# wenlinlee/FISCO-BCOS

Measured on AMD Instinct MI355X. Metric: sigs_per_sec, higher is better.
Workload: dtype u32 (256-bit integer); 1 GPU; C2; txs_total=10000, txs_rank0=10000, parallelism=dp1 (tx-index shards)

## Files before the change

### fisco-bcos_amd/csrc/ecc_coop.hip

```cpp
#include "ecc_device.h"
#include "ec26_trio.h"

namespace bcosgpu {

struct SplitLds {
    uint32_t tab[8][16][64];
    uint32_t zc[8][64];
    uint32_t u1[8][64];
    uint32_t k1[4][64];
    uint32_t k2[4][64];
    uint32_t flags[64];
    uint32_t pt[3][25][64];
};

__device__ __forceinline__ void lds_store_jac(uint32_t (*dst)[64], const Jac& P, int lane) {
    lds_store_fe(dst, P.X, lane);
    lds_store_fe(dst + 8, P.Y, lane);
    lds_store_fe(dst + 16, P.Z, lane);
    dst[24][lane] = P.inf ? 1u : 0u;
}
__device__ __forceinline__ void lds_load_jac(Jac& P, const uint32_t (*src)[64], int lane) {
    lds_load_fe(P.X, src, lane);
    lds_load_fe(P.Y, src + 8, lane);
    lds_load_fe(P.Z, src + 16, lane);
    P.inf = src[24][lane] != 0u;
}

__device__ __forceinline__ void add_digit_lds(Jac& acc, const SplitLds& L, int lane, int d, bool neg, bool phi) {
    const uint32_t m = static_cast<uint32_t>((d < 0 ? -d : d) - 1) & 7u;
    const uint32_t* base = &L.tab[0][0][0] + m * (16 * 64) + lane;
    Aff S;
#pragma unroll
    for (int k = 0; k < 8; ++k) {
        S.x.v[k] = base[k * 64];
        S.y.v[k] = base[(8 + k) * 64];
    }
    if (phi) {
        fe b;
        fe_set(b, kGlvBeta);
        FieldK1::mul(S.x, S.x, b);
    }
    fe ny;
    FieldK1::neg(ny, S.y);
    fe_cmov(S.y, ny, (d < 0) != neg);
    Jac R;
    CurveK1::madd(R, acc, S);
    CurveK1::cmov(acc, R, d != 0);
}

__device__ __forceinline__ void glv_half_lds(Jac& acc, fe& k, bool neg, bool phi, const SplitLds& L, int lane) {
    CurveK1::set_inf(acc);
    add_digit_lds(acc, L, lane, static_cast<int>(k.v[3] >> 31), neg, phi);
#pragma unroll 1
    for (int i = 31; i >= 0; --i) {
        CurveK1::dbl(acc, acc);
        CurveK1::dbl(acc, acc);
        CurveK1::dbl(acc, acc);
        CurveK1::dbl(acc, acc);
        add_digit_lds(acc, L, lane, booth_digit128(k), neg, phi);
    }
}

__global__ __launch_bounds__(256, 1) void tx_verify_split_kernel(const uint8_t* __restrict__ pre,
                                                                 const uint64_t* __restrict__ pre_off,
                                                                 const uint8_t* __restrict__ sig,
                                                                 const uint64_t* __restrict__ sig_off, uint64_t n,
                                                                 const uint32_t* __restrict__ tab,
                                                                 uint8_t* __restrict__ txhash,
                                                                 uint8_t* __restrict__ sender,
                                                                 uint8_t* __restrict__ status) {
    __shared__ SplitLds L;
    const int wave = threadIdx.x >> 6, lane = threadIdx.x & 63;
    const uint64_t i = static_cast<uint64_t>(blockIdx.x) * 64 + lane;
    const bool active = i < n;
    uint64_t sa = 0, sb = 0;
    if (active) {
        sa = sig_off[i];
        sb = sig_off[i + 1];
    }
    const uint32_t slen = (sb - sa) > 0xffffffffull ? 0xffffffffu : static_cast<uint32_t>(sb - sa);
    if (wave == 1) {
        if (active) {
            const uint64_t a = pre_off[i], b = pre_off[i + 1];
            const uint32_t len = static_cast<uint32_t>(b - a);
            ByteReader rd(pre + a, len);
            uint32_t d[8];
            keccak256_msg(rd, len, d);
            store_digest(KECCAK256, txhash + 32 * i, d);
            fe e, r, s;
            uint32_t v;
            fe_from_be_words(e, d);
            reduce_once(e, ParamN1::M);
            const bool ok = parse_sig65(sig + sa, slen, r, s, v);
            if (!ok) {
                fe_zero(r);
                r.v[0] = 1;
                fe_zero(s);
            }
            fe rm, rinv, u1, u2, k1, k2;
            FieldN1::from_plain(rm, r);
            FieldInv<FieldN1>::inv(rinv, rm);
            FieldN1::mul(u1, e, rinv);
            FieldN1::neg(u1, u1);
            FieldN1::mul(u2, s, rinv);
            bool neg1, neg2;
            glv_split(k1, neg1, k2, neg2, u2);
            lds_store_fe(L.u1, u1, lane);
#pragma unroll
            for (int k = 0; k < 4; ++k) {
                L.k1[k][lane] = k1.v[k];
                L.k2[k][lane] = k2.v[k];
            }
            L.flags[lane] = (ok ? 1u : 0u) | (neg1 ? 4u : 0u) | (neg2 ? 8u : 0u);
        }
    } else if (wave == 2) {
        if (active) {
            fe r, s;
            uint32_t v;
            bool ok = parse_sig65(sig + sa, slen, r, s, v);
            fe x;
            fe_copy(x, r);
            if (v & 2u) {
                ok = ok && fe_lt_k(r, kK1PminusN);
                fe_add_k(x, r, ParamN1::M);
            }
            fe rhs, y, t, seven;
            FieldK1::sqr(t, x);
            FieldK1::mul(rhs, t, x);
            fe_zero(seven);
            seven.v[0] = 7;
            FieldK1::add(rhs, rhs, seven);
            FieldK1::sqrt_cand(y, rhs);
            FieldK1::sqr(t, y);
            ok = ok && FieldK1::eq(t, rhs);
            FieldK1::normalize(y);
            fe ny;
            FieldK1::neg(ny, y);
            FieldK1::normalize(ny);
            fe_cmov(y, ny, (y.v[0] & 1u) != (v & 1u));
            Aff R, A[8];
            fe_copy(R.x, x);
            fe_copy(R.y, y);
            fe Zc;
            {
                Jac T[8];
                multiples8<CurveK1>(T, R);
                coz_table_k1(A, Zc, T);
            }
            Unroll<0, 8>::run([&](auto J) {
                constexpr int j = decltype(J)::value;
                lds_store_fe(L.tab[j], A[j].x, lane);
                lds_store_fe(L.tab[j] + 8, A[j].y, lane);
            });
            lds_store_fe(L.zc, Zc, lane);
            L.pt[2][24][lane] = ok ? 2u : 0u;
        }
    }
    __syncthreads();
    uint32_t flags = 0;
    if (active) flags = L.flags[lane] | L.pt[2][24][lane];
    __syncthreads();
    if (wave <= 1) {
        if (active) {
            fe k;
            fe_zero(k);
#pragma unroll
            for (int q = 0; q < 4; ++q) k.v[q] = wave == 0 ? L.k1[q][lane] : L.k2[q][lane];
            const bool neg = wave == 0 ? (flags & 4u) != 0 : (flags & 8u) != 0;
            Jac P;
            glv_half_lds(P, k, neg, wave == 1, L, lane);
            lds_store_jac(L.pt[wave], P, lane);
        }
    } else if (wave == 2) {
        if (active) {
            fe u1;
            lds_load_fe(u1, L.u1, lane);
            Jac PG;
            comb_mul<CurveK1, 8>(PG, u1, tab);
            lds_store_jac(L.pt[2], PG, lane);
        }
    }
    __syncthreads();
    if (wave == 0 && active) {
        Jac P0, P1, PG, Q, R;
        lds_load_jac(P0, L.pt[0], lane);
        lds_load_jac(P1, L.pt[1], lane);
        lds_load_jac(PG, L.pt[2], lane);
        fe Zc;
        lds_load_fe(Zc, L.zc, lane);
        CurveK1::add(Q, P0, P1);
        FieldK1::mul(Q.Z, Q.Z, Zc);
        CurveK1::add(R, Q, PG);
        const bool ok = (flags & 3u) == 3u && !R.inf;
        Aff A;
        CurveK1::to_aff(A, R);
        FieldK1::normalize(A.x);
        FieldK1::normalize(A.y);
        uint32_t ad[5] = {0, 0, 0, 0, 0};
        if (ok) keccak_address(ad, A.x, A.y);
        uint32_t* o = reinterpret_cast<uint32_t*>(sender + 20 * i);
#pragma unroll
        for (int k = 0; k < 5; ++k) o[k] = ad[k];
        status[i] = ok ? 0 : 1;
    }
}

#ifdef BCOSGPU_COOP_TIMING
__device__ uint64_t g_coop_t[8][12];
__device__ uint64_t g_dbl_t[4][8];
#define DBL_T(k) \
    if (c.probe && (threadIdx.x & 63) == 0) g_dbl_t[threadIdx.x >> 6][k] = clock64()
#define COOP_T(k) \
    if (blockIdx.x == 0 && (threadIdx.x & 63) == 0) g_coop_t[threadIdx.x >> 6][k] = clock64()
#else
#define COOP_T(k) \
    do {          \
    } while (0)
#define DBL_T(k) \
    do {         \
    } while (0)
#endif
struct CoopLds {
    uint32_t tab[8][16][64];
    uint32_t zc[8][64];
    uint32_t k[2][4][64];
    uint32_t flags[64];
    uint4 ex[2][2][6][2][64];
    uint32_t tabphx[8][8][64];
    uint32_t pt[5][25][64];
    uint32_t xe[8][64];
    uint32_t xrinv[8][64];
    uint32_t ys[8][64];
    uint32_t rflag[64];
    uint32_t post[2];
};

struct CoopCtx {
    CoopLds* L;
    int chain, role, lane;
    bool probe;
    __device__ __forceinline__ uint4* slot(int x, int r, int f) const {
        return &L->ex[chain][r][x == 0 ? f : 2 + x][0][0] + lane;
    }
    __device__ __forceinline__ void put(int x, int f, const fe& a) const {
        uint4* p = slot(x, role, f);
        p[0] = make_uint4(a.v[0], a.v[1], a.v[2], a.v[3]);
        p[64] = make_uint4(a.v[4], a.v[5], a.v[6], a.v[7]);
    }
    __device__ __forceinline__ void puts(int s, const fe& a) const {
        uint4* p = &L->ex[chain][role][s][0][0] + lane;
        p[0] = make_uint4(a.v[0], a.v[1], a.v[2], a.v[3]);
        p[64] = make_uint4(a.v[4], a.v[5], a.v[6], a.v[7]);
    }
    __device__ __forceinline__ void gets(int s, fe& a) const {
        const uint4* p = &L->ex[chain][role ^ 1][s][0][0] + lane;
        const uint4 q0 = p[0], q1 = p[64];
        a.v[0] = q0.x; a.v[1] = q0.y; a.v[2] = q0.z; a.v[3] = q0.w;
        a.v[4] = q1.x; a.v[5] = q1.y; a.v[6] = q1.z; a.v[7] = q1.w;
    }
    __device__ __forceinline__ void get(int x, int f, fe& a) const {
        const uint4* p = slot(x, role ^ 1, f);
        const uint4 q0 = p[0], q1 = p[64];
        a.v[0] = q0.x; a.v[1] = q0.y; a.v[2] = q0.z; a.v[3] = q0.w;
        a.v[4] = q1.x; a.v[5] = q1.y; a.v[6] = q1.z; a.v[7] = q1.w;
    }
};

template <int S0>
__device__ __forceinline__ void coop_dbl(Jac& P, const CoopCtx& c) {
    fe E, F, D, C8, Z3, X3, Y3, t;
    DBL_T(0);
    if (c.role == 0) {
        fe A;
        FieldK1::sqr(A, P.X);
        FieldK1::mul3(E, A);
        FieldK1::sqr(F, E);
        c.puts(S0, E);
        c.puts(S0 + 1, F);
        FieldK1::mul(Z3, P.Y, P.Z);
        FieldK1::template shl<1>(Z3, Z3);
        c.puts(S0 + 2, Z3);
    } else {
        fe B, C;
        FieldK1::sqr(B, P.Y);
        FieldK1::mul(D, P.X, B);
        FieldK1::template shl<2>(D, D);
        c.puts(S0, D);
        FieldK1::sqr(C, B);
        FieldK1::template shl<3>(C8, C);
        c.puts(S0 + 1, C8);
    }
    DBL_T(1);
    __syncthreads();
    DBL_T(2);
    if (c.role == 0) {
        c.gets(S0, D);
        c.gets(S0 + 1, C8);
    } else {
        c.gets(S0, E);
        c.gets(S0 + 1, F);
        c.gets(S0 + 2, Z3);
    }
    FieldK1::template shl<1>(t, D);
    FieldK1::sub(X3, F, t);
// ... 829 lines not shown
    if (wave == 1) {
        fe u2, k1, k2;
        FieldN1::mul(u2, VERIFY ? r : s, rinv);
        bool neg1, neg2;
        glv_split(k1, neg1, k2, neg2, u2);
#pragma unroll
        for (int q = 0; q < 4; ++q) {
            L.k[0][q][lane] = k1.v[q];
            L.k[1][q][lane] = k2.v[q];
        }
        L.flags[lane] = (ok ? 1u : 0u) | (neg1 ? 4u : 0u) | (neg2 ? 8u : 0u);
    }
}

struct CombShare {
    int wide[4][2], narrow[4][2];
};
__device__ __forceinline__ void comb_share(int& lo, int& hi, const int (&t)[4][2], int wave) {
    lo = t[0][0];
    hi = t[0][1];
#pragma unroll
    for (int w = 1; w < 4; ++w) {
        if (wave == w) {
            lo = t[w][0];
            hi = t[w][1];
        }
    }
}
__device__ __forceinline__ void comb_share_range(Jac26& G, const fe& u1, const uint32_t* __restrict__ tab, int tab_bits,
                                                 const CombShare& share, int wave) {
    int lo, hi;
    if (tab_bits == kWideBits) {
        comb_share(lo, hi, share.wide, wave);
        comb_range26w<kWideBits>(G, u1, tab, lo, hi);
    } else {
        comb_share(lo, hi, share.narrow, wave);
        comb_range26w<8>(G, u1, tab, lo, hi);
    }
}
constexpr int kPairShare[4][2] = {{0, 12}, {24, 32}, {0, 0}, {12, 24}};
constexpr int kTrioSplitWin[3] = {5, 10, 16};
static_assert(0 < kTrioSplitWin[0] && kTrioSplitWin[0] < kTrioSplitWin[1] && kTrioSplitWin[1] < kTrioSplitWin[2] &&
                  kTrioSplitWin[2] <= 16,
              "comb windows of helpers 0, 1, 3, 2");
constexpr CombShare trio_recover_share() {
    const int a = kTrioSplitWin[0], b = kTrioSplitWin[1], c = kTrioSplitWin[2];
    return {{{0, a}, {a, b}, {c, 16}, {b, c}}, {{0, 2 * a}, {2 * a, 2 * b}, {2 * c, 32}, {2 * b, 2 * c}}};
}
constexpr CombShare kTrioRecoverShare = trio_recover_share();
constexpr CombShare kTrioVerifyShare = {{{0, 6}, {15, 16}, {10, 15}, {6, 10}}, {{0, 11}, {30, 32}, {19, 30}, {11, 19}}};

template <class LDS>
__device__ __forceinline__ void coop26_store_partial(LDS& L, const Jac26& G, int wave, int lane) {
    if (wave == 0) {
        coop26_store_jac(L.pt[2], G, lane);
        lds_flag_post(&L.post[2]);
    } else if (wave == 3) {
        Jac26 G0, S;
        lds_flag_wait(&L.post[2]);
        coop26_load_jac(G0, L.pt[2], lane);
        CurveK1x::add(S, G0, G);
        coop26_store_jac(L.pt[3], S, lane);
    } else {
        coop26_store_jac(L.pt[wave == 1 ? 4 : 0], G, lane);
    }
}

template <class IO>
__device__ __forceinline__ void coop26_body(const IO& io, uint64_t n, const uint32_t* __restrict__ tab) {
    __shared__ Coop26Lds L;
    const int wave = threadIdx.x >> 6, lane = threadIdx.x & 63;
    const uint64_t i = static_cast<uint64_t>(blockIdx.x) * 64 + lane;
    const bool active = i < n;
    COOP_T(0);
    if (threadIdx.x == 0) {
        L.post[0] = 0u;
        L.post[1] = 0u;
        L.post[2] = 0u;
    }
    __syncthreads();
    fe r, s;
    uint32_t v = 0;
    bool ok = false;
    if (active) ok = io.rsv(i, r, s, v);
    else { fe_zero(r); fe_zero(s); }
    if (wave == 1 || wave == 2) {
        fe26 X, rhs;
        bool okr = recover_w(X, rhs, r, v, ok);
        if (wave == 2) {
            fe26 y, ny, t;
            fe26_sqrt_cand(y, rhs);
            fe26_sqr(t, y);
            fe26_sub<3>(t, t, rhs);
            okr = okr && fe26_is_zero(t);
            fe26_normalize(y);
            fe26_neg<2>(ny, y);
            fe26_normalize(ny);
            fe26_cmov(y, ny, (y.v[0] & 1u) != (v & 1u));
            lds_store_fe26(L.ys, y, lane);
            L.rflag[lane] = okr ? 2u : 0u;
            COOP_T(6);
        } else {
            Aff26 R;
            fe26_mul(R.x, rhs, X);
            fe26_sqr(R.y, rhs);
            coop26_table_to_lds<false>(L, R, lane);
            COOP_T(6);
        }
    }
    coop26_post_e_inv<false, false>(L, io, i, active, ok, r, s, wave, lane);
    if (wave != 2) {
        fe u1;
        coop26_u1_glv<false>(u1, L, ok, r, s, wave, lane);
        Jac26 G;
        int lo, hi;
        comb_share(lo, hi, kPairShare, wave);
        comb_range26w<8>(G, u1, tab, lo, hi);
        coop26_store_partial(L, G, wave, lane);
    }
    COOP_T(1);
    __syncthreads();
    const uint32_t flags = L.flags[lane] | L.rflag[lane];
    {
        Coop26Ctx c{&L, wave >> 1, wave & 1, lane, false};
        fe k;
        fe_zero(k);
#pragma unroll
        for (int q = 0; q < 4; ++q) k.v[q] = L.k[c.chain][q][lane];
        const bool neg = c.chain == 0 ? (flags & 4u) != 0 : (flags & 8u) != 0;
        const bool phi = c.chain == 1;
        Jac26 acc;
        CurveK1x::set_inf(acc);
        coop26_add_digit(acc, c, static_cast<int>(k.v[3] >> 31), neg, phi);
#pragma unroll 1
        for (int w = 31; w >= 0; --w) {
            coop26_dbl<0>(acc, c);
#ifdef BCOSGPU_COOP_TIMING
            c.probe = blockIdx.x == 0 && w == 20;
#endif
            coop26_dbl<3>(acc, c);
#ifdef BCOSGPU_COOP_TIMING
            c.probe = false;
            if (blockIdx.x == 0 && w == 20 && (threadIdx.x & 63) == 0) g_dbl_t[threadIdx.x >> 6][5] = clock64();
#endif
            coop26_dbl<0>(acc, c);
            coop26_dbl<3>(acc, c);
#ifdef BCOSGPU_COOP_TIMING
            if (blockIdx.x == 0 && w == 20 && (threadIdx.x & 63) == 0) g_dbl_t[threadIdx.x >> 6][6] = clock64();
#endif
            coop26_add_digit(acc, c, booth_digit128(k), neg, phi);
#ifdef BCOSGPU_COOP_TIMING
            if (blockIdx.x == 0 && w == 20 && (threadIdx.x & 63) == 0) g_dbl_t[threadIdx.x >> 6][7] = clock64();
#endif
        }
        COOP_T(2);
        if (c.role == 0) coop26_store_jac(L.pt[c.chain], acc, lane);
    }
    __syncthreads();
    if (wave == 1) {
        Jac26 G01, G2, U;
        coop26_load_jac(G01, L.pt[3], lane);
        coop26_load_jac(G2, L.pt[4], lane);
        CurveK1x::add(U, G01, G2);
        coop26_store_jac(L.pt[2], U, lane);
    } else if (wave == 0) {
        Jac26 P0, P1, Q;
        coop26_load_jac(P0, L.pt[0], lane);
        coop26_load_jac(P1, L.pt[1], lane);
        fe26 Zc, y;
        lds_load_fe26(Zc, L.zc, lane);
        lds_load_fe26(y, L.ys, lane);
        CurveK1x::add(Q, P0, P1);
        fe26_mul(Zc, Zc, y);
        fe26_mul(Q.Z, Q.Z, Zc);
        coop26_store_jac(L.pt[0], Q, lane);
    }
    __syncthreads();
    if (wave == 0 && active) {
        Jac26 Q, G, R;
        coop26_load_jac(Q, L.pt[0], lane);
        coop26_load_jac(G, L.pt[2], lane);
        CurveK1x::add(R, Q, G);
        const bool ok2 = (flags & 3u) == 3u && !R.inf;
        COOP_T(4);
        fe z, zi, ax, ay;
        fe26_to_fe(z, R.Z);
        FieldInv<FieldK1>::inv(zi, z);
        COOP_T(5);
        fe26 zi26, zi2, zi3, X, Y;
        fe26_from_fe(zi26, zi);
        fe26_sqr(zi2, zi26);
        fe26_mul(X, R.X, zi2);
        fe26_mul(zi3, zi2, zi26);
        fe26_mul(Y, R.Y, zi3);
        fe26_to_fe(ax, X);
        fe26_to_fe(ay, Y);
        uint32_t ad[5] = {0, 0, 0, 0, 0};
        if (ok2 && io.want_addr()) keccak_address(ad, ax, ay);
        io.finish(i, ok2, ad, &ax, &ay);
    }
    COOP_T(3);
}

constexpr int kTrioTxs = 40;
struct TrioSeat {
    int chain, tl;
    bool real;
    __device__ __forceinline__ TrioSeat(int wave, int lane, const TrioLane& T) {
        const int trio_idx = (lane & 15) / 3;
        chain = wave & 1;
        tl = (wave >> 1) * 20 + (lane >> 4) * 5 + (trio_idx < 5 ? trio_idx : 4);
        real = T.r2 && trio_idx < 5;
    }
};

template <class IO>
__device__ __forceinline__ void trio_recover_tail(const IO& io, uint32_t* mbuf, int wave, int lane, const TrioSeat& seat,
                                                  uint64_t ti, bool tactive, bool ok2, const fe& ax, const fe& ay) {
    if (seat.chain == 0 && io.want_addr()) {
        const KeccakPair kp;
        const int j = lane >> 1, t = (wave >> 1) * 20 + (j < 20 ? j : 0);
        uint32_t d[4];
        kp.hash(reinterpret_cast<const uint8_t*>(mbuf + 16 * t), 64u, d);
        if (j < 20) {
#pragma unroll
            for (int q = 0; q < 4; ++q) mbuf[640 + 8 * t + 2 * q + (lane & 1)] = d[q];
        }
    }
    __syncthreads();
    if (seat.chain == 0 && seat.real && tactive) {
        uint32_t ad[5] = {0, 0, 0, 0, 0};
        if (ok2 && io.want_addr()) {
#pragma unroll
            for (int q = 0; q < 5; ++q) ad[q] = mbuf[640 + 8 * seat.tl + 3 + q];
        }
        io.finish(ti, ok2, ad, &ax, &ay);
    }
}

__device__ __forceinline__ void lds_flag_wait_idle(uint32_t* f) {
    while (__hip_atomic_load(f, __ATOMIC_ACQUIRE, __HIP_MEMORY_SCOPE_WORKGROUP) == 0u) __builtin_amdgcn_s_sleep(8);
}

template <class IO>
__device__ __forceinline__ void trio_recover_helper(Trio26RecoverLds& L, const IO& io, uint64_t i, bool active, bool ok,
                                                    const fe& r, uint32_t v, const uint32_t* __restrict__ tab, int tab_bits,
                                                    int h, int lane) {
    constexpr bool kRootAdds = kTrioSplitWin[2] < 16;
    constexpr int kLast = kRootAdds ? 3 : 2;
    if (h == 2) {
        fe26 X, w, y, ny, t;
        const bool okr = recover_w(X, w, r, v, ok);
        fe26_sqrt_cand(y, w);
        fe26_sqr(t, y);
        fe26_sub<3>(t, t, w);
        const bool on = fe26_is_zero(t);
        fe26_normalize(y);
        fe26_neg<2>(ny, y);
        fe26_normalize(ny);
        fe26_cmov(y, ny, (y.v[0] & 1u) != (v & 1u));
        if (lane < kTrioTxs) {
#pragma unroll
            for (int q = 0; q < 10; ++q) L.sq[q][lane] = y.v[q];
        }
        L.rflag[lane] = okr ? 2u : 0u;
        L.yok[lane] = on ? 1u : 0u;
        COOP_T(6);
    } else if (h == 3) {
        fe e;
        fe_zero(e);
        if (active) io.template digest<KECCAK256>(i, e);
        reduce_once(e, ParamN1::M);
        lds_store_fe(L.xe, e, lane);
        lds_flag_post(&L.post[1]);
        COOP_T(7);
    }
    int lo, hi;
    comb_share(lo, hi, kTrioRecoverShare.wide, h);
    if (lo != hi) {
        lds_flag_wait_idle(&L.post[0]);
        lds_flag_wait_idle(&L.post[1]);
        fe e, rinv, u1;
        lds_load_fe(e, L.xe, lane);
        lds_load_fe(rinv, L.xrinv, lane);
        FieldN1::mul(u1, e, rinv);
        FieldN1::neg(u1, u1);
        Jac26 G;
        comb_share_range(G, u1, tab, tab_bits, kTrioRecoverShare, h);
        const int j = h == 0 ? 0 : h == 1 ? 1 : h == 3 ? 2 : 3;
        if (j > 0) {
            Jac26 P, S;
            lds_flag_wait_idle(&L.hpost[j - 1]);
            coop26_load_jac(P, L.pt[j - 1], lane);
            CurveK1x::add(S, P, G);
            coop26_store_jac(L.pt[j == kLast ? 3 : j], S, lane);
        } else {
            coop26_store_jac(L.pt[0], G, lane);
        }
        if (j != kLast) lds_flag_post(&L.hpost[j]);
        COOP_T(10);
    }
}

template <class IO>
__device__ __forceinline__ void trio26_recover_body(const IO& io, uint64_t n, const uint32_t* __restrict__ tab,
                                                    int tab_bits) {
    __shared__ Trio26RecoverLds L;
    const int wave = __builtin_amdgcn_readfirstlane(static_cast<int>(threadIdx.x >> 6)), lane = threadIdx.x & 63;
    const bool helper = wave >= 4;
    const uint64_t i = static_cast<uint64_t>(blockIdx.x) * kTrioTxs + lane;
    const bool active = lane < kTrioTxs && i < n;
    COOP_T(0);
    if (threadIdx.x == 0) {
        L.post[0] = 0u;
        L.post[1] = 0u;
        L.post[2] = 0u;
#pragma unroll
        for (int q = 0; q < kTfSlots; ++q) L.spost[q] = 0u;
#pragma unroll
        for (int q = 0; q < 4; ++q) L.hpost[q] = 0u;
    }
    __syncthreads();
    const TrioLane T(lane);
    TrioSeat seat(wave, lane, T);
    if (helper) seat.chain = 2;
    const int chain = seat.chain, tl = seat.tl;
    uint32_t tflags = 0;
    TrioPt acc;
    {
        fe r, s;
        uint32_t v = 0;
        bool ok = false;
        fe_zero(r);
        fe_zero(s);
        if (active && (wave <= 3 || wave == 4 + 2)) ok = io.rsv(i, r, s, v);
        if (helper) {
            trio_recover_helper(L, io, i, active, ok, r, v, tab, tab_bits, wave - 4, lane);
            COOP_T(1);
        } else {
            if (wave == 0) {
                if (!ok) {
                    fe_zero(r);
                    r.v[0] = 1;
                    fe_zero(s);
                }
                fe rm, rinv, u2, k1, k2;
                FieldN1::from_plain(rm, r);
                FieldInv<FieldN1>::inv_pipe(rinv, rm);
                lds_store_fe(L.xrinv, rinv, lane);
                lds_flag_post(&L.post[0]);
                COOP_T(7);
                FieldN1::mul(u2, s, rinv);
                COOP_T(10);
                bool neg1, neg2;
                glv_split(k1, neg1, k2, neg2, u2);
                COOP_T(11);
#pragma unroll
                for (int q = 0; q < 4; ++q) {
                    L.k[0][q][lane] = k1.v[q];
                    L.k[1][q][lane] = k2.v[q];
                }
                L.flags[lane] = (ok ? 1u : 0u) | (neg1 ? 4u : 0u) | (neg2 ? 8u : 0u);
                lds_flag_post(&L.spost[0]);
                COOP_T(8);
            } else {
                fe26 X, rhs, beta;
                recover_w(X, rhs, r, v, ok);
                Aff26 R;
                fe26_mul(R.x, rhs, X);
                fe26_sqr(R.y, rhs);
                fe26_const(beta, kGlvBeta);
                TrioTableFlags tf{L.spost};
                if (wave == 1) trio_table_shared<kTableLong>(L, tf, R, rhs, beta, lane);
                else if (wave == 2) trio_table_shared<kTablePrefix>(L, tf, R, rhs, beta, lane);
                else trio_table_shared<kTableShort>(L, tf, R, rhs, beta, lane);
            }
            COOP_T(1);
            lds_flag_wait4(&L.spost[0], &L.spost[kTfDone[kTableLong]], &L.spost[kTfDone[kTablePrefix]],
                           &L.spost[kTfDone[kTableShort]]);
            COOP_T(9);
            tflags = L.flags[tl];
            trio_glv_chain(acc, L, chain, tl, tflags, T);
            COOP_T(2);
        }
    }
    uint32_t* const xbuf = &L.xg[(wave >> 1) & 1][0][0];
    uint32_t* const mbuf = &L.tabphx[0][0][0];
    const uint64_t ti = static_cast<uint64_t>(blockIdx.x) * kTrioTxs + tl;
    const bool tactive = ti < n;
    fe ax, ay;
    bool ok2 = false;
    const auto load_k = [&](fe26& K) {
#pragma unroll
        for (int q = 0; q < 10; ++q) K.v[q] = L.kw[q][tl];
        F26_SETM(K, 1);
    };
    const auto load_g = [&](TrioPt& G) {
        Jac26 J;
        coop26_load_jac(J, L.pt[3], tl);
        trio_from_jac(G, J, T);
    };
    TrioPt SE;
    fe26 zi2, zi3;
    fe26_zero(zi2);
    fe26_zero(zi3);
    if (chain == 1) {
        trio_store(xbuf, acc, lane);
        lds_flag_post(&L.spost[5 + (wave >> 1)]);
    } else if (chain == 0) {
        TrioPt P1;
        lds_flag_wait(&L.spost[5 + (wave >> 1)]);
        trio_load(P1, xbuf, lane);
        trio_add(acc, acc, P1, T);
        trio_store(xbuf, acc, lane);
        fe26 K;
        load_k(K);
        trio_scale_xz(SE, acc, K, T);
    }
    __syncthreads();
    const uint32_t rfl = L.rflag[tl];
    if (chain == 0) {
        TrioPt G;
        load_g(G);
        fe26 Z3;
        trio_add_z(Z3, G, SE, T);
        COOP_T(4);
        fe z, zi;
        fe26_to_fe(z, Z3);
        FieldInv<FieldK1>::inv_trio<2, 2>(zi, z, T, lane);
        COOP_T(5);
        fe26 zi26;
        fe26_from_fe(zi26, zi);
        fe26_sqr(zi2, zi26);
        fe26_mul(zi3, zi2, zi26);
    } else if (chain == 1) {
        TrioPt S, G;
        trio_load(S, xbuf, lane);
        load_g(G);
        fe26 y, zc, K, l;
        load_k(K);
        lds_load_fe26(zc, L.zc, tl);
        trio_scale_xz(SE, S, K, T);
#pragma unroll
        for (int q = 0; q < 10; ++q) y.v[q] = L.sq[q][tl];
        F26_SETM(y, 1);
        COOP_T(4);
        fe26_mul(l, zc, y);
        trio_scale_y(SE, l, T);
        trio_add(S, G, SE, T);
        trio_store(xbuf, S, lane);
        COOP_T(5);
    }
    __syncthreads();
    if (chain == 0) {
        TrioPt O;
        trio_load(O, xbuf, lane);
        ok2 = (tflags & 1u) != 0u && (rfl & 2u) != 0u && L.yok[tl] != 0u && !O.inf;
        fe26 X, Y;
        fe26_mul(X, O.Xs, zi2);
        fe26_mul(Y, O.S1, zi3);
        fe26_to_fe(ax, X);
        fe26_to_fe(ay, Y);
        if (seat.real) {
            uint32_t m[16];
            fe_to_be_words(m, ax);
            fe_to_be_words(m + 8, ay);
#pragma unroll
            for (int q = 0; q < 16; ++q) mbuf[16 * tl + q] = m[q];
        }
    }
    __syncthreads();
    trio_recover_tail(io, mbuf, wave, lane, seat, ti, tactive, ok2, ax, ay);
    COOP_T(3);
}

__device__ __forceinline__ void trio26_verify_body(const KeyIO& io, uint64_t n, const uint32_t* __restrict__ tab,
                                                   int tab_bits) {
    __shared__ Trio26Lds L;
    const int wave = threadIdx.x >> 6, lane = threadIdx.x & 63;
    const uint64_t i = static_cast<uint64_t>(blockIdx.x) * kTrioTxs + lane;
    const bool active = lane < kTrioTxs && i < n;
    COOP_T(0);
    if (threadIdx.x == 0) {
        L.post[0] = 0u;
        L.post[1] = 0u;
        L.post[2] = 0u;
    }
    __syncthreads();
    fe r, s;
    bool ok = false;
    {
        fe kx, ky;
        if (active) {
            io.key_rs(i, r, s, kx, ky);
            ok = fe_lt_k(kx, FieldK1::P) && fe_lt_k(ky, FieldK1::P) && !fe_is_zero_raw(r) && !fe_is_zero_raw(s) &&
                 fe_lt_k(r, ParamN1::M) && fe_lt_k(s, kN1HalfPlus);
        } else {
            fe_zero(r);
            fe_zero(s);
            fe_zero(kx);
            fe_zero(ky);
        }
        if (wave == 0) lds_store_fe(L.ys, r, lane);
        if (wave == 1) {
            Aff26 P;
            fe26_from_fe(P.x, kx);
            fe26_from_fe(P.y, ky);
            fe26 l, rr, t, seven;
            fe26_sqr(l, P.y);
            fe26_sqr(t, P.x);
            fe26_mul(rr, t, P.x);
            fe26_set_small(seven, 7u);
            fe26_add(rr, rr, seven);
            fe26_sub<3>(l, l, rr);
            const bool on = fe26_is_zero(l);
            if (!(ok && on)) {
                fe26_const(P.x, kK1Gx);
                fe26_const(P.y, kK1Gy);
            }
            L.rflag[lane] = on ? 2u : 0u;
            coop26_table_to_lds<true>(L, P, lane);
            COOP_T(6);
        }
    }
    coop26_post_e_inv<true, true>(L, io, i, active, ok, r, s, wave, lane);
    {
        fe u1;
        coop26_u1_glv<true>(u1, L, ok, r, s, wave, lane);
        Jac26 G;
        comb_share_range(G, u1, tab, tab_bits, kTrioVerifyShare, wave);
        coop26_store_partial(L, G, wave, lane);
    }
    COOP_T(1);
    __syncthreads();
    const TrioLane T(lane);
    const TrioSeat seat(wave, lane, T);
    const int chain = seat.chain, tl = seat.tl;
    const uint32_t tflags = L.flags[tl] | L.rflag[tl];
    TrioPt acc;
    trio_glv_chain(acc, L, chain, tl, tflags, T);
    COOP_T(2);
    uint32_t* const xbuf = &L.tab[0][0][0] + (wave >> 1) * kTrioWords * 64;
    uint32_t* const gbuf = &L.tab[0][0][0] + (2 + (wave >> 1)) * kTrioWords * 64;
    const uint64_t ti = static_cast<uint64_t>(blockIdx.x) * kTrioTxs + tl;
    fe26 zcy;
    bool ok2 = false;
    __syncthreads();
    if (chain == 1) trio_store(xbuf, acc, lane);
    else lds_load_fe26(zcy, L.zc, tl);
    __syncthreads();
    if (chain == 1) {
        TrioPt A;
        trio_sum_partials<true, false>(A, L, tl, T);
        trio_store(gbuf, A, lane);
    } else {
        TrioPt P1;
        trio_load(P1, xbuf, lane);
        trio_add(acc, acc, P1, T);
        fe26_mul(acc.Zs, acc.Zs, zcy);
    }
    __syncthreads();
    if (chain == 0) {
        TrioPt G;
        trio_load(G, gbuf, lane);
        trio_add(acc, acc, G, T);
        fe rr, r2, xw, cw;
        lds_load_fe(rr, L.ys, tl);
        fe26 z2, c, rhs;
        fe26_sqr(z2, acc.Zs);
        fe26_from_fe(c, rr);
        fe26_mul(rhs, c, z2);
        fe26_to_fe(xw, acc.Xs);
        fe26_to_fe(cw, rhs);
        bool match = fe_eq_raw(xw, cw);
        const uint32_t carry = fe_add_k(r2, rr, ParamN1::M);
        const bool second = carry == 0u && fe_lt_k(r2, FieldK1::P);
        fe26_from_fe(c, second ? r2 : rr);
        fe26_mul(rhs, c, z2);
        fe26_to_fe(cw, rhs);
        match = match || (second && fe_eq_raw(xw, cw));
        ok2 = (tflags & 3u) == 3u && !acc.inf && match;
    }
    __syncthreads();
    __syncthreads();
    if (chain == 0 && seat.real && ti < n) {
        const uint32_t ad[5] = {0, 0, 0, 0, 0};
        io.finish(ti, ok2, ad, nullptr, nullptr);
    }
    COOP_T(3);
}

template <class IO>
__global__ __launch_bounds__(256, 1) void tx_verify_coop26_kernel(IO io, uint64_t n, const uint32_t* __restrict__ tab) {
    coop26_body(io, n, tab);
}

constexpr int kTrioRecoverThreads = 512;
template <class IO>
__global__ __launch_bounds__(kTrioRecoverThreads, 2) void tx_verify_trio26_kernel(IO io, uint64_t n, const uint32_t* __restrict__ tab,
                                                                  int tab_bits) {
    trio26_recover_body(io, n, tab, tab_bits);
}

__global__ __launch_bounds__(256, 1) void sig_verify_trio26_kernel(KeyIO io, uint64_t n, const uint32_t* __restrict__ tab,
                                                                   int tab_bits) {
    trio26_verify_body(io, n, tab, tab_bits);
}

int launch_sig_verify_small_secp(const KeyIO& io, uint64_t n, hipStream_t st) {
    const uint32_t *k1, *sm2;
    int bits = 8;
    const int rc = tables(&k1, &sm2, &bits);
    if (rc) return rc;
    hipLaunchKernelGGL(sig_verify_trio26_kernel, dim3(static_cast<unsigned>((n + 39) / 40)), dim3(256), 0, st, io, n, k1,
                       bits);
    return hipGetLastError() == hipSuccess ? 0 : BCOSGPU_E_HIP;
}


template <class IO>
int launch_verify_small_secp(const TxKernelPolicy& pol, const IO& io, uint64_t n, hipStream_t st) {
    if (pol.coop == 3 && pol.f26) return launch_recover_row(io, n, st);
    const uint32_t *k1, *sm2;
    const int rc = tables8(&k1, &sm2);
    if (rc) return rc;
    const dim3 grid(static_cast<unsigned>((n + 63) / 64));
    if (pol.coop == 2 && pol.f26) {
        const uint32_t *wk1, *wsm2;
        int bits = 8;
        const int rw = tables(&wk1, &wsm2, &bits);
        if (rw) return rw;
        hipLaunchKernelGGL(tx_verify_trio26_kernel<IO>, dim3(static_cast<unsigned>((n + 39) / 40)),
                           dim3(kTrioRecoverThreads), 0, st, io, n, wk1, bits);
    } else if (pol.coop && pol.f26) {
        hipLaunchKernelGGL(tx_verify_coop26_kernel<IO>, grid, dim3(256), 0, st, io, n, k1);
    } else if constexpr (std::is_same_v<IO, TxIO>) {
        if (pol.coop)
            hipLaunchKernelGGL(tx_verify_coop_kernel, grid, dim3(256), 0, st, io.pre, io.pre_off, io.sig, io.sig_off, n,
                               k1, io.txhash, io.sender, io.status);
        else
            hipLaunchKernelGGL(tx_verify_split_kernel, grid, dim3(256), 0, st, io.pre, io.pre_off, io.sig, io.sig_off,
                               n, k1, io.txhash, io.sender, io.status);
    } else {
        return BCOSGPU_E_ARG;
    }
    return hipGetLastError() == hipSuccess ? 0 : BCOSGPU_E_HIP;
}
template int launch_verify_small_secp<TxIO>(const TxKernelPolicy&, const TxIO&, uint64_t, hipStream_t);
template int launch_verify_small_secp<SigIO>(const TxKernelPolicy&, const SigIO&, uint64_t, hipStream_t);
template int launch_verify_small_secp<EcrecIO>(const TxKernelPolicy&, const EcrecIO&, uint64_t, hipStream_t);

}
```

### fisco-bcos_amd/csrc/ecc_txv.hip

```cpp
#include "ecc_device.h"

namespace bcosgpu {

template <int SUITE, int OCC, bool F26, class IO>
__global__ __launch_bounds__(256, OCC) void tx_verify_kernel(IO io, uint64_t n, const uint32_t* __restrict__ tab,
                                                             int tbits) {
    const uint64_t i = static_cast<uint64_t>(blockIdx.x) * blockDim.x + threadIdx.x;
    if (i >= n) return;
    fe h;
    io.template digest<SUITE == BCOSGPU_SUITE_SM2 ? SM3 : KECCAK256>(i, h);
    fe x, y, r, s;
    uint32_t ad[5] = {0, 0, 0, 0, 0};
    bool ok;
    constexpr bool kLds = OCC == 2;
    __shared__ uint32_t ldsx_all[kLds ? 4 * 4096 : 1];
    uint32_t* ldsx = kLds ? ldsx_all + (threadIdx.x >> 6) * 4096 + (threadIdx.x & 63) : nullptr;
    if constexpr (SUITE == BCOSGPU_SUITE_SM2 && std::is_same_v<IO, KeyIO>) {
        uint32_t X[8], Y[8];
        io.sm2_sig(i, r, s, X, Y);
        if constexpr (F26) ok = sm2_verify_rs26<kLds>(h, r, s, X, Y, CombTab{tab, tbits}, x, y, ldsx);
        else ok = sm2_verify_rs<kLds>(h, r, s, X, Y, CombTab{tab, tbits}, x, y, ldsx);
        io.finish(i, ok, ad, nullptr, nullptr);
    } else if constexpr (SUITE == BCOSGPU_SUITE_SM2) {
        const uint8_t* sp;
        const uint32_t slen = io.sig_span(i, sp);
        if constexpr (F26) ok = sm2_verify_lane26<kLds>(h, sp, slen, CombTab{tab, tbits}, x, y, ldsx);
        else ok = sm2_verify_lane<kLds>(h, sp, slen, CombTab{tab, tbits}, x, y, ldsx);
        if (ok && io.want_addr()) sm3_address(ad, x, y);
        io.finish(i, ok, ad, nullptr, nullptr);
    } else {
        uint32_t v;
        io.rsv(i, r, s, v);
        if constexpr (F26) ok = secp256k1_recover_rsv26<kLds>(h, r, s, v, CombTab{tab, tbits}, x, y, ldsx);
        else ok = secp256k1_recover_rsv<kLds>(h, r, s, v, CombTab{tab, tbits}, x, y, ldsx);
        if (ok && io.want_addr()) keccak_address(ad, x, y);
        io.finish(i, ok, ad, &x, &y);
    }
}

static constexpr double kRowLat = 0.38, kRowLatN = 0.18;
static constexpr double kRowLatSM2 = 0.43, kRowLatNSM2 = 0.14;
static constexpr uint64_t kRowResidentSM2 = 4;
static int auto_kernel(int suite, uint64_t n, int cus, bool small_ok, bool row_ok) {
    const bool sm2 = suite == BCOSGPU_SUITE_SM2;
    const double lat[4] = {sm2 ? 4.315 : 4.475, sm2 ? 2.399 : 2.643, sm2 ? 1.678 : 1.279, 1.0};
    const double occ2_tail = sm2 ? 2.452 : 2.556;
    const uint64_t per[4] = {512ull * cus, 256ull * cus, 64ull * cus, 40ull * cus};
    const int code[4] = {-2, 0, 1, 2};
    int best = 0;
    double cost = 1e300;
    for (int k = small_ok ? 3 : 1; k >= 0; --k) {
        double c = static_cast<double>((n + per[k] - 1) / per[k]) * lat[k];
        if (k == 0) {
            const uint64_t tail = n % per[0];
            c = static_cast<double>(n / per[0]) * lat[0] + (tail == 0 ? 0.0 : tail <= per[1] ? occ2_tail : lat[0]);
        }
        if (c < cost) {
            cost = c;
            best = code[k];
        }
    }
    if (row_ok && small_ok) {
        const double r1 = sm2 ? kRowLatSM2 : kRowLat, rn = sm2 ? kRowLatNSM2 : kRowLatN;
        const uint64_t m = (n + cus - 1) / cus, res = sm2 ? kRowResidentSM2 : m;
        const uint64_t rounds = (m + res - 1) / res;
        const double c = static_cast<double>(rounds) * r1 + static_cast<double>(m - rounds) * rn;
        if (c < cost) best = 3;
    }
    return best;
}

template <class IO>
int launch_verify(int suite, const IO& io, uint64_t n, hipStream_t st) {
    if (n == 0) return 0;
    const uint32_t *k1, *sm2;
    int bits;
    int rc = tables(&k1, &sm2, &bits);
    if (rc) return rc;
    TxKernelPolicy pol = tx_policy();
    constexpr bool kTx = std::is_same_v<IO, TxIO>;
    bool small = pol.split >= 0 ? pol.split == 1 : n <= (1ull << 15);
    int occ = pol.occ;
    if (pol.split < 0 && pol.coop == 2 && pol.f26) {
        static const bool row_env = [] {
            const char* e = getenv("BCOSGPU_TXV_ROW");
            return !(e && atoi(e) == 0);
        }();
        const bool row_io = suite == BCOSGPU_SUITE_SM2 || !std::is_same_v<IO, KeyIO>;
        const int k = auto_kernel(suite, n, cu_count(), n <= (1ull << 16), row_env && row_io);
        small = k > 0;
        if (small) pol.coop = k;
        else if (!occ) occ = k == -2 ? 2 : 1;
    }
    if (!occ) occ = n >= (1ull << 17) ? 2 : 1;
    if (small && !kTx && !(pol.f26 && pol.coop)) small = false;
    constexpr bool kK1 = !std::is_same_v<IO, KeyIO>, kSM2 = !std::is_same_v<IO, EcrecIO>;
    if constexpr (kK1)
        if (suite == BCOSGPU_SUITE_SECP256K1 && small) return launch_verify_small_secp(pol, io, n, st);
    if constexpr (kSM2)
        if (suite == BCOSGPU_SUITE_SM2 && small && pol.coop) return launch_verify_small_sm2(pol, io, n, st);
#define TXV(S, O, F, T) \
    hipLaunchKernelGGL((tx_verify_kernel<S, O, F, IO>), dim3(grid_of(n)), dim3(256), 0, st, io, n, T, bits)
    if (suite == BCOSGPU_SUITE_SM2) {
        if constexpr (kSM2) {
            if (pol.f26) {
                const uint32_t* t26;
                rc = tables_sm2_26(&t26, &bits);
                if (rc) return rc;
                if (occ == 2) TXV(BCOSGPU_SUITE_SM2, 2, true, t26); else TXV(BCOSGPU_SUITE_SM2, 1, true, t26);
            } else {
                if (occ == 2 && kTx) TXV(BCOSGPU_SUITE_SM2, 2, false, sm2); else TXV(BCOSGPU_SUITE_SM2, 1, false, sm2);
            }
        } else {
            return BCOSGPU_E_ARG;
        }
    } else if constexpr (kK1) {
        if (pol.f26) {
            if (occ == 2) TXV(BCOSGPU_SUITE_SECP256K1, 2, true, k1); else TXV(BCOSGPU_SUITE_SECP256K1, 1, true, k1);
        } else {
            if (occ == 2 && kTx) TXV(BCOSGPU_SUITE_SECP256K1, 2, false, k1); else TXV(BCOSGPU_SUITE_SECP256K1, 1, false, k1);
        }
    } else {
        return BCOSGPU_E_ARG;
    }
#undef TXV
    return hipGetLastError() == hipSuccess ? 0 : BCOSGPU_E_HIP;
}

int launch_tx_verify(int suite, const uint8_t* d_pre, const uint64_t* d_pre_off, const uint8_t* d_sig,
                     const uint64_t* d_sig_off, uint64_t n, uint8_t* d_txhash, uint8_t* d_sender, uint8_t* d_status,
                     hipStream_t st) {
    const TxIO io{d_pre, d_pre_off, d_sig, d_sig_off, d_txhash, d_sender, d_status};
    return launch_verify(suite, io, n, st);
}

int launch_secp256k1_recover(const uint8_t* d_hash, const uint8_t* d_sig, uint32_t stride, uint64_t n, uint8_t* d_pub,
                             uint8_t* d_addr, uint8_t* d_ok, hipStream_t st) {
    const SigIO io{d_hash, d_sig, stride, 65u, d_pub, d_addr, d_ok};
    return launch_verify(BCOSGPU_SUITE_SECP256K1, io, n, st);
}

int launch_sm2_verify(const uint8_t* d_hash, const uint8_t* d_sig, uint32_t stride, uint64_t n, uint8_t* d_addr,
                      uint8_t* d_ok, hipStream_t st) {
    const SigIO io{d_hash, d_sig, stride, 128u, nullptr, d_addr, d_ok};
    return launch_verify(BCOSGPU_SUITE_SM2, io, n, st);
}

int launch_ecrecover(const uint8_t* d_in, uint64_t n, uint8_t* d_out, uint8_t* d_ok, hipStream_t st) {
    const EcrecIO io{d_in, d_out, d_ok};
    return launch_verify(BCOSGPU_SUITE_SECP256K1, io, n, st);
}

int launch_sm2_verify_key(const uint8_t* d_pub, const uint8_t* d_hash, const uint8_t* d_sig, uint32_t stride,
                          uint64_t n, uint8_t* d_ok, hipStream_t st) {
    const KeyIO io{d_pub, d_hash, d_sig, stride, d_ok};
    return launch_verify(BCOSGPU_SUITE_SM2, io, n, st);
}
}
```

Measured before the change: 32.21 million tx/s (hash + recover/verify + sender).

## Pair r and s inversions across trio lanes in recover wave zero

Wave 0 of the trio recover kernel now loads signatures with a remapped lane-to-transaction layout. It computes r^-1 and s*r^-1 by multiplying paired values across neighbouring lanes via DPP shifts, then does one cooperative trio modular inversion instead of a per-lane inv_pipe. The scalar k1/k2 results are posted before rinv, so the table waves can start earlier. The auto-kernel cost model also discounts the trio path for secp256k1, which makes it more likely to be picked. This adds cross-lane shuffles, extra multiplies and phantom lanes, and the outcome depends on getting the role and column mapping right.

```diff
diff --git a/fisco-bcos_amd/csrc/ecc_coop.hip b/fisco-bcos_amd/csrc/ecc_coop.hip
--- a/fisco-bcos_amd/csrc/ecc_coop.hip
+++ b/fisco-bcos_amd/csrc/ecc_coop.hip
@@ -1,5 +1,6 @@
 #include "ecc_device.h"
 #include "ec26_trio.h"
+#include "pair_inv.h"
 
 namespace bcosgpu {
 
@@ -1435,6 +1436,45 @@
     }
 }
 
+struct PairOpsTrio {
+    const TrioLane& T;
+    int lane;
+    template <int CTRL>
+    __device__ __forceinline__ static void shift(fe& o, const fe& a) {
+#pragma unroll
+        for (int q = 0; q < 8; ++q) o.v[q] = trio::dpp<CTRL>(a.v[q]);
+    }
+    __device__ __forceinline__ void right1(fe& o, const fe& a) const { shift<trio::kR1>(o, a); }
+    __device__ __forceinline__ void left1(fe& o, const fe& a) const { shift<trio::kL1>(o, a); }
+    __device__ __forceinline__ void left2(fe& o, const fe& a) const { shift<trio::kL2>(o, a); }
+    __device__ __forceinline__ void sel(fe& o, int roles, const fe& a, const fe& b) const {
+        const bool c = ((roles & kPairRole0) && T.r0) || ((roles & kPairRole1) && T.r1) || ((roles & kPairRole2) && T.r2);
+#pragma unroll
+        for (int q = 0; q < 8; ++q) o.v[q] = c ? a.v[q] : b.v[q];
+    }
+    __device__ __forceinline__ void mul(fe& o, const fe& a, const fe& b) const {
+        FieldN1::mul(o, a, b);
+        asm volatile("s_nop 1"
+                     : "+v"(o.v[0]), "+v"(o.v[1]), "+v"(o.v[2]), "+v"(o.v[3]), "+v"(o.v[4]), "+v"(o.v[5]), "+v"(o.v[6]),
+                       "+v"(o.v[7]));
+    }
+    __device__ __forceinline__ void inv(fe& o, const fe& x) const {
+        fe t, a, b;
+        modinv_trio<0, 1>(t, x, kMod30N1, T, lane);
+        shift<trio::kR1>(a, t);
+        shift<trio::kL1>(b, t);
+#pragma unroll
+        for (int q = 0; q < 8; ++q) o.v[q] = T.r1 ? t.v[q] : T.r0 ? a.v[q] : b.v[q];
+    }
+    __device__ __forceinline__ void stamp(int k) const {
+        if (k == kPairStampPre) {
+            COOP_T(6);
+        } else {
+            COOP_T(10);
+        }
+    }
+};
+
 template <class IO>
 __device__ __forceinline__ void trio26_recover_body(const IO& io, uint64_t n, const uint32_t* __restrict__ tab,
                                                     int tab_bits) {
@@ -1466,36 +1506,40 @@
         bool ok = false;
         fe_zero(r);
         fe_zero(s);
-        if (active && (wave <= 3 || wave == 4 + 2)) ok = io.rsv(i, r, s, v);
+        if (wave != 0 && active && (wave <= 3 || wave == 4 + 2)) ok = io.rsv(i, r, s, v);
         if (helper) {
             trio_recover_helper(L, io, i, active, ok, r, v, tab, tab_bits, wave - 4, lane);
             COOP_T(1);
         } else {
             if (wave == 0) {
-                if (!ok) {
-                    fe_zero(r);
-                    r.v[0] = 1;
-                    fe_zero(s);
-                }
-                fe rm, rinv, u2, k1, k2;
-                FieldN1::from_plain(rm, r);
-                FieldInv<FieldN1>::inv_pipe(rinv, rm);
-                lds_store_fe(L.xrinv, rinv, lane);
-                lds_flag_post(&L.post[0]);
-                COOP_T(7);
-                FieldN1::mul(u2, s, rinv);
-                COOP_T(10);
+                const bool phantom = (lane & 15) == 15, member = !T.r2 && !phantom;
+                const int col = phantom ? 60 + (lane >> 4) : tl + (T.r1 ? 20 : T.r2 ? 40 : 0);
+                const uint64_t i0 = static_cast<uint64_t>(blockIdx.x) * kTrioTxs + col;
+                if (member && i0 < n) ok = io.rsv(i0, r, s, v);
+                pair_enter(r, s, ok);
+                PairOpsTrio ops{T, lane};
+                fe u2, inv, rinv, k1, k2;
+                pair_scalars(u2, inv, r, s, ops);
                 bool neg1, neg2;
                 glv_split(k1, neg1, k2, neg2, u2);
                 COOP_T(11);
-#pragma unroll
-                for (int q = 0; q < 4; ++q) {
-                    L.k[0][q][lane] = k1.v[q];
-                    L.k[1][q][lane] = k2.v[q];
+                if (member) {
+#pragma unroll
+                    for (int q = 0; q < 4; ++q) {
+                        L.k[0][q][col] = k1.v[q];
+                        L.k[1][q][col] = k2.v[q];
+                    }
+                    L.flags[col] = (ok ? 1u : 0u) | (neg1 ? 4u : 0u) | (neg2 ? 8u : 0u);
                 }
-                L.flags[lane] = (ok ? 1u : 0u) | (neg1 ? 4u : 0u) | (neg2 ? 8u : 0u);
                 lds_flag_post(&L.spost[0]);
                 COOP_T(8);
+                pair_rinv(rinv, inv, r, ops);
+                fe one;
+                fe_set(one, ParamN1::ONE);
+                fe_cmov(rinv, one, !member);
+                lds_store_fe(L.xrinv, rinv, col);
+                lds_flag_post(&L.post[0]);
+                COOP_T(7);
             } else {
                 fe26 X, rhs, beta;
                 recover_w(X, rhs, r, v, ok);
diff --git a/fisco-bcos_amd/csrc/ecc_txv.hip b/fisco-bcos_amd/csrc/ecc_txv.hip
--- a/fisco-bcos_amd/csrc/ecc_txv.hip
+++ b/fisco-bcos_amd/csrc/ecc_txv.hip
@@ -41,6 +41,7 @@
 static constexpr double kRowLat = 0.38, kRowLatN = 0.18;
 static constexpr double kRowLatSM2 = 0.43, kRowLatNSM2 = 0.14;
 static constexpr uint64_t kRowResidentSM2 = 4;
+static constexpr double kTrioRoundK1 = 0.796;
 static int auto_kernel(int suite, uint64_t n, int cus, bool small_ok, bool row_ok) {
     const bool sm2 = suite == BCOSGPU_SUITE_SM2;
     const double lat[4] = {sm2 ? 4.315 : 4.475, sm2 ? 2.399 : 2.643, sm2 ? 1.678 : 1.279, 1.0};
@@ -51,6 +52,7 @@
     double cost = 1e300;
     for (int k = small_ok ? 3 : 1; k >= 0; --k) {
         double c = static_cast<double>((n + per[k] - 1) / per[k]) * lat[k];
+        if (k == 3 && !sm2) c *= kTrioRoundK1;
         if (k == 0) {
             const uint64_t tail = n % per[0];
             c = static_cast<double>(n / per[0]) * lat[0] + (tail == 0 ? 0.0 : tail <= per[1] ? occ2_tail : lat[0]);
diff --git a/fisco-bcos_amd/csrc/pair_inv.h b/fisco-bcos_amd/csrc/pair_inv.h
--- /dev/null
+++ b/fisco-bcos_amd/csrc/pair_inv.h
@@ -0,0 +1,57 @@
+#pragma once
+#include <stdint.h>
+
+#include "fe26.h"
+
+#if defined(__HIPCC__) || defined(__HIP__)
+#define PAIR_TABLE __device__ __constant__ static const uint32_t
+#else
+#define PAIR_TABLE static const uint32_t
+#endif
+
+namespace bcosgpu {
+
+PAIR_TABLE kPairR2N1[8] = {0x67d7d140u, 0x896cf214u, 0x0e7cf878u, 0x741496c2u,
+                           0x5bcd07c6u, 0xe697f5e4u, 0x81c69bc5u, 0x9d671cd5u};
+
+constexpr int kPairRole0 = 1, kPairRole1 = 2, kPairRole2 = 4;
+constexpr int kPairStampPre = 0, kPairStampInv = 1;
+
+template <class V>
+F26_HD void pair_enter(V& r, V& s, bool ok) {
+#pragma unroll
+    for (int i = 0; i < 8; ++i) {
+        r.v[i] = ok ? r.v[i] : (i == 0 ? 1u : 0u);
+        s.v[i] = ok ? s.v[i] : 0u;
+    }
+}
+
+template <class V, class Ops>
+F26_HD void pair_scalars(V& u2, V& inv, const V& r, const V& s, Ops& ops) {
+    V rr1, rl2, sl1, x, y, pre, t, k;
+    ops.right1(rr1, r);
+    ops.left2(rl2, r);
+    ops.left1(sl1, s);
+    ops.sel(x, kPairRole2, rl2, r);
+    ops.sel(y, kPairRole0, rr1, sl1);
+    ops.mul(pre, x, y);
+    ops.stamp(kPairStampPre);
+    ops.inv(t, pre);
+#pragma unroll
+    for (int i = 0; i < 8; ++i) k.v[i] = kPairR2N1[i];
+    ops.mul(inv, t, k);
+    ops.stamp(kPairStampInv);
+    ops.right1(y, pre);
+    ops.mul(u2, inv, y);
+}
+
+template <class V, class Ops>
+F26_HD void pair_rinv(V& rinv, const V& inv, const V& r, Ops& ops) {
+    V rr1, rl1, y;
+    ops.right1(rr1, r);
+    ops.left1(rl1, r);
+    ops.sel(y, kPairRole0, rr1, rl1);
+    ops.mul(rinv, inv, y);
+}
+
+}
```

Measured after the change: 33.05 million tx/s (hash + recover/verify + sender) (median of 6 runs). 2.6% higher.
